# MDFahimAnjum/AliasFree-Diffusion-Models-PyTorch

Hardware: AMD Instinct MI355X
Metric: train_step_images_per_sec (higher is better)
Workload: dtype f32; 1 GPU; CIFAR-10 32x32x3 synthetic, UNet variant=3 (Config D), batch 256/GPU, T=1000, AdamW lr 3e-4, random-init weights (seed 42); global_batch=256, parallelism=dp1, hip_graph=True, launch_mode=lanes

## Files before the change

aliasfree-diffusion-models-pytorch_amd/csrc/tok.hip:

```cpp
#include "common.h"
#include <algorithm>
#include <cstdint>
#include <mutex>
#include <set>

namespace afd {

using f32x16 = __attribute__((ext_vector_type(16))) float;

template <int NB> struct TT { f32x16 b[NB]; };

__device__ __forceinline__ constexpr int tch(int j, int r) { return 32 * j + (r & 3) + 8 * (r >> 2); }

struct Pix { unsigned b, p, f; bool live; };
__device__ __forceinline__ Pix pix_of(int tile, int l31, unsigned total, unsigned P) {
  Pix q;
  q.f = (unsigned)tile * 32u + (unsigned)l31;
  q.live = q.f < total;
  const unsigned fc = q.live ? q.f : 0u;
  q.b = fc / P;
  q.p = fc - q.b * P;
  return q;
}
__device__ __forceinline__ unsigned tbase(const Pix& q, unsigned Cx, unsigned P, int half) {
  return q.b * Cx * P + q.p + 4u * (unsigned)half * P;
}

template <int NB>
__device__ __forceinline__ void t_load(TT<NB>& z, const float* __restrict__ src, unsigned base, unsigned P, bool live) {
#pragma unroll
  for (int j = 0; j < NB; ++j)
#pragma unroll
    for (int r = 0; r < 16; ++r) z.b[j][r] = live ? src[base + (unsigned)tch(j, r) * P] : 0.f;
}
template <int NB>
__device__ __forceinline__ void t_store(const TT<NB>& z, float* __restrict__ dst, unsigned base, unsigned P, bool live) {
  if (!live) return;
#pragma unroll
  for (int j = 0; j < NB; ++j)
#pragma unroll
    for (int r = 0; r < 16; ++r) dst[base + (unsigned)tch(j, r) * P] = z.b[j][r];
}

template <int KB>
__device__ __forceinline__ f32x16 t_block(const float* __restrict__ Ws, int nb, int l31, int half, const TT<KB>& z, f32x16 acc) {
  constexpr int WS = 32 * KB + 4;
  const float* __restrict__ wr = Ws + (nb * 32 + l31) * WS + 4 * half;
#pragma unroll
  for (int j = 0; j < KB; ++j)
#pragma unroll
    for (int q = 0; q < 4; ++q) {
      const float4 a = *reinterpret_cast<const float4*>(wr + 32 * j + 8 * q);
      acc = __builtin_amdgcn_mfma_f32_32x32x2f32(a.x, z.b[j][4 * q + 0], acc, 0, 0, 0);
      acc = __builtin_amdgcn_mfma_f32_32x32x2f32(a.y, z.b[j][4 * q + 1], acc, 0, 0, 0);
      acc = __builtin_amdgcn_mfma_f32_32x32x2f32(a.z, z.b[j][4 * q + 2], acc, 0, 0, 0);
      acc = __builtin_amdgcn_mfma_f32_32x32x2f32(a.w, z.b[j][4 * q + 3], acc, 0, 0, 0);
    }
  return acc;
}
__device__ __forceinline__ f32x16 zero16() {
  f32x16 a;
#pragma unroll
  for (int r = 0; r < 16; ++r) a[r] = 0.f;
  return a;
}

template <int K>
__device__ __forceinline__ void stage_w(float* __restrict__ Ws, const float* __restrict__ w, int rows, int ldw, int n0, int k0,
                                        bool transposed) {
  constexpr int WS = K + 4;
  if (!transposed) {
    for (int i = threadIdx.x; i < rows * K; i += 256) {
      const int n = i / K, k = i - n * K;
      Ws[n * WS + k] = w[(long)(n0 + n) * ldw + k0 + k];
    }
  } else {
    for (int i = threadIdx.x; i < rows * K; i += 256) {
      const int n = i / K, k = i - n * K;
      Ws[n * WS + k] = w[(long)(k0 + k) * ldw + n0 + n];
    }
  }
}

template <int KB>
__device__ __forceinline__ void t_ln_fwd(const TT<KB>& x, const float* __restrict__ gs, const float* __restrict__ bs, int half,
                                         float eps, TT<KB>& y, float& mean, float& rstd) {
  constexpr float invC = 1.0f / (32 * KB);
  float s = 0.f;
#pragma unroll
  for (int j = 0; j < KB; ++j)
#pragma unroll
    for (int r = 0; r < 16; ++r) s += x.b[j][r];
  s += __shfl_xor(s, 32, 64);
  mean = s * invC;
  float q = 0.f;
#pragma unroll
  for (int j = 0; j < KB; ++j)
#pragma unroll
    for (int r = 0; r < 16; ++r) { const float d = x.b[j][r] - mean; q = fmaf(d, d, q); }
  q += __shfl_xor(q, 32, 64);
  rstd = 1.0f / sqrtf(q * invC + eps);
#pragma unroll
  for (int j = 0; j < KB; ++j)
#pragma unroll
    for (int r = 0; r < 16; ++r) {
      const int c = tch(j, r) + 4 * half;
      y.b[j][r] = (x.b[j][r] - mean) * rstd * gs[c] + bs[c];
    }
}
template <int KB>
__device__ __forceinline__ void t_ln_bwd(TT<KB>& dy, const TT<KB>& x, const float* __restrict__ gs, int half, float mean,
                                         float rstd, const TT<KB>& add) {
  constexpr float invC = 1.0f / (32 * KB);
  float s1 = 0.f, s2 = 0.f;
#pragma unroll
  for (int j = 0; j < KB; ++j)
#pragma unroll
    for (int r = 0; r < 16; ++r) {
      const float gv = gs[tch(j, r) + 4 * half] * dy.b[j][r];
      const float xh = (x.b[j][r] - mean) * rstd;
      dy.b[j][r] = gv;
      s1 += gv;
      s2 = fmaf(gv, xh, s2);
    }
  s1 += __shfl_xor(s1, 32, 64);
  s2 += __shfl_xor(s2, 32, 64);
  const float m1 = s1 * invC, m2 = s2 * invC;
#pragma unroll
  for (int j = 0; j < KB; ++j)
#pragma unroll
    for (int r = 0; r < 16; ++r) {
      const float xh = (x.b[j][r] - mean) * rstd;
      dy.b[j][r] = rstd * (dy.b[j][r] - m1 - xh * m2) + add.b[j][r];
    }
}

template <int C>
__global__ __launch_bounds__(256) void tok_head_fwd(const float* __restrict__ x, const float* __restrict__ gamma,
                                                    const float* __restrict__ beta, const float* __restrict__ w,
                                                    const float* __restrict__ bias, float* __restrict__ h_out,
                                                    float* __restrict__ stats_out, float* __restrict__ y, int B, int N, int P,
                                                    float eps, int n_per_wg) {
  constexpr int KB = C / 32, WS = C + 4;
  extern __shared__ __attribute__((aligned(16))) float smem[];
  float* Ws = smem;
  float* bsm = Ws + n_per_wg * WS;
  float* gs = bsm + n_per_wg;
  float* bes = gs + C;
  const int nbase = blockIdx.y * n_per_wg;
  stage_w<C>(Ws, w, n_per_wg, C, nbase, 0, false);
  for (int i = threadIdx.x; i < n_per_wg; i += 256) bsm[i] = bias ? bias[nbase + i] : 0.f;
  for (int i = threadIdx.x; i < C; i += 256) { gs[i] = gamma[i]; bes[i] = beta[i]; }
  __syncthreads();

  const int lane = threadIdx.x & 63, wv = threadIdx.x >> 6, half = lane >> 5, l31 = lane & 31;
  const unsigned total = (unsigned)B * (unsigned)P;
  const int ntile = (int)((total + 31u) / 32u);
  const int tstride = gridDim.x * 4;
  const bool lead = blockIdx.y == 0;
  const int nblk = n_per_wg / 32;

  TT<KB> xc, xn;
  Pix pc, pn;
  int t = blockIdx.x * 4 + wv;
  if (t < ntile) { pc = pix_of(t, l31, total, P); t_load(xc, x, tbase(pc, C, P, half), P, pc.live); }
  for (; t < ntile; t += tstride) {
    const int tn = t + tstride;
    if (tn < ntile) { pn = pix_of(tn, l31, total, P); t_load(xn, x, tbase(pn, C, P, half), P, pn.live); }
    TT<KB> h;
    float mean, rstd;
    t_ln_fwd<KB>(xc, gs, bes, half, eps, h, mean, rstd);
    if (lead) {
      if (h_out) t_store(h, h_out, tbase(pc, C, P, half), P, pc.live);
      if (stats_out && pc.live && half == 0) { stats_out[2 * pc.f] = mean; stats_out[2 * pc.f + 1] = rstd; }
    }
    const unsigned yb = tbase(pc, N, P, half);
    for (int nb = 0; nb < nblk; ++nb) {
      const f32x16 acc = t_block<KB>(Ws, nb, l31, half, h, zero16());
      if (pc.live) {
#pragma unroll
        for (int r = 0; r < 16; ++r) {
          const int nl = nb * 32 + tch(0, r) + 4 * half;
          y[yb + (unsigned)(nbase + nb * 32 + tch(0, r)) * (unsigned)P] = acc[r] + bsm[nl];
        }
      }
    }
    xc = xn; pc = pn;
  }
}

template <int C> struct Chain {
  static constexpr int KB = C / 32, WS = C + 4, SLOT = C * WS;
  static constexpr bool RELOAD = C > 64;
  static constexpr int NSLOT = RELOAD ? 2 : 3;
};

template <int C, bool TRAIN>
__global__ __launch_bounds__(256) void tok_tail_fwd(const float* __restrict__ att, const float* __restrict__ xres,
                                                    const float* __restrict__ wo, const float* __restrict__ bo,
                                                    const float* __restrict__ gamma, const float* __restrict__ beta,
                                                    const float* __restrict__ w1, const float* __restrict__ b1,
                                                    const float* __restrict__ w2, const float* __restrict__ b2,
                                                    float* __restrict__ a_out, float* __restrict__ stats_out,
                                                    float* __restrict__ f_out, float* __restrict__ u_out, float* __restrict__ g_out,
                                                    float* __restrict__ out, int B, int P, float eps) {
  using CH = Chain<C>;
  constexpr int KB = CH::KB;
  extern __shared__ __attribute__((aligned(16))) float smem[];
  float* s0 = smem;
  float* s1 = smem + CH::SLOT;
  float* s2 = CH::RELOAD ? s0 : smem + 2 * CH::SLOT;
  float* vec = smem + CH::NSLOT * CH::SLOT;
  stage_w<C>(s0, wo, C, C, 0, 0, false);
  stage_w<C>(s1, w1, C, C, 0, 0, false);
  if (!CH::RELOAD) stage_w<C>(s2, w2, C, C, 0, 0, false);
  for (int i = threadIdx.x; i < C; i += 256) {
    vec[i] = bo[i]; vec[C + i] = gamma[i]; vec[2 * C + i] = beta[i]; vec[3 * C + i] = b1[i]; vec[4 * C + i] = b2[i];
// ... 459 lines not shown
  x_put(Xt, nbk, l31, half, dfb);
  __syncthreads();
  x_get<KB>(Xt, l31, half, z);
  const float mean = pc.live ? stats[2 * pc.f] : 0.f, rstd = pc.live ? stats[2 * pc.f + 1] : 0.f;
  float m1, m2;
  t_ln_bwd_core<KB>(z, aa, gs, half, mean, rstd, m1, m2);
  t_load(aa, dout, base, P, pc.live);
#pragma unroll
  for (int j = 0; j < KB; ++j)
#pragma unroll
    for (int r = 0; r < 16; ++r) z.b[j][r] += aa.b[j][r];
  {
    const f32x16 ab = b_load(a_in, bb, P, pc.live), dob = b_load(dout, bb, P, pc.live);
    f32x16 dab;
#pragma unroll
    for (int r = 0; r < 16; ++r) {
      const float xh = (ab[r] - mean) * rstd;
      dab[r] = rstd * (gs[cb + tch(0, r)] * dfb[r] - m1 - xh * m2) + dob[r];
    }
    b_store(dab, da_out, bb, P, pc.live);
  }
  const f32x16 db = wa_block<KB>(wa, z, zero16());
  b_store(db, datt_out, bb, P, pc.live);
}

template <int C>
__global__ __launch_bounds__(256) void tok_head_bwd_wide(const float* __restrict__ dqkv, const float* __restrict__ x,
                                                         const float* __restrict__ stats, const float* __restrict__ gamma,
                                                         const float* __restrict__ w_in, const float* __restrict__ dres,
                                                         float* __restrict__ dh_out, float* __restrict__ dx_out, int B, int P) {
  using WD = Wide<C>;
  constexpr int KB = WD::KB;
  __shared__ float X[WD::TPW][C * 32];
  __shared__ float gs[C];
  for (int i = threadIdx.x; i < C; i += 256) gs[i] = gamma[i];
  const int lane = threadIdx.x & 63, wv = threadIdx.x >> 6, half = lane >> 5, l31 = lane & 31;
  const int ts = wv / WD::NS, nbk = wv % WD::NS;
  const unsigned total = (unsigned)B * (unsigned)P;
  const int ntile = (int)((total + 31u) / 32u);
  const int tile = blockIdx.x * WD::TPW + ts;
  const bool active = tile < ntile;
  Pix pc = pix_of(active ? tile : 0, l31, total, P);
  pc.live = pc.live && active;
  const unsigned base = tbase(pc, C, P, half), bb = base + (unsigned)(nbk * 32) * (unsigned)P;
  const unsigned qb = tbase(pc, 3 * C, P, half);
  const int cb = nbk * 32 + 4 * half;
  float* Xt = X[ts];
  TT<KB> z;
  WA<KB> wa;
  f32x16 dhb = zero16();
#pragma unroll
  for (int sct = 0; sct < 3; ++sct) {
    t_load(z, dqkv, qb + (unsigned)(sct * C) * (unsigned)P, P, pc.live);
    wa_load_t(wa, w_in, nbk * 32, C, sct * C, l31, half);
    dhb = wa_block<KB>(wa, z, dhb);
  }
  if (dh_out) b_store(dhb, dh_out, bb, P, pc.live);
  x_put(Xt, nbk, l31, half, dhb);
  TT<KB> xx;
  t_load(xx, x, base, P, pc.live);
  __syncthreads();
  x_get<KB>(Xt, l31, half, z);
  const float mean = pc.live ? stats[2 * pc.f] : 0.f, rstd = pc.live ? stats[2 * pc.f + 1] : 0.f;
  float m1, m2;
  t_ln_bwd_core<KB>(z, xx, gs, half, mean, rstd, m1, m2);
  const f32x16 xb = b_load(x, bb, P, pc.live), rb = b_load(dres, bb, P, pc.live);
  f32x16 dxb;
#pragma unroll
  for (int r = 0; r < 16; ++r) {
    const float xh = (xb[r] - mean) * rstd;
    dxb[r] = rstd * (gs[cb + tch(0, r)] * dhb[r] - m1 - xh * m2) + rb[r];
  }
  b_store(dxb, dx_out, bb, P, pc.live);
}

static bool tok_ok(int C) { return C == 32 || C == 64 || C == 128; }
static size_t chain_lds(int C, int nvec) {
  const int nslot = C > 64 ? 2 : 3;
  return sizeof(float) * ((size_t)nslot * C * (C + 4) + (size_t)nvec * C);
}
template <class K> static int set_lds(K kern, size_t lds) { return lds_opt_in(kern, lds); }
static int g_tok_max_wg = 0;
static int g_tok_path = 0;
static bool use_wide(int C, long ntile) {
  if (C != 64 && C != 128) return false;
  if (g_tok_max_wg > 0 || g_tok_path == 1) return false;
  if (g_tok_path == 2) return true;
  return C == 128 || ntile < 1024;
}
static unsigned chain_grid(int C, long ntile) {
  const long wg = (ntile + 3) / 4;
  const long cap = g_tok_max_wg > 0 ? g_tok_max_wg : (C > 64 ? 8192 : 1024);
  return (unsigned)std::min<long>(wg, cap);
}

}

using namespace afd;

extern "C" {

int afd_tok_supported(int C) { return tok_ok(C) ? 1 : 0; }
int afd_debug_tok_grid(int max_workgroups) { g_tok_max_wg = max_workgroups; return AFD_OK; }
int afd_debug_tok_path(int mode) { g_tok_path = mode; return AFD_OK; }

int afd_tok_head_fwd(const float* x, const float* gamma, const float* beta, const float* w, const float* bias, float* h_out,
                     float* stats_out, float* qkv, int B, int C, int P, float eps, afd_stream_t st) {
  AFD_REQUIRE(x && gamma && beta && w && qkv && B > 0 && P > 0, "afd_tok_head_fwd: NULL pointer or empty shape");
  AFD_REQUIRE(tok_ok(C), "afd_tok_head_fwd: C=%d not covered (32, 64, 128)", C);
  AFD_REQUIRE((long)B * P * 3 * C < (1L << 31), "afd_tok_head_fwd: tensor too large for 32-bit offsets");
  const int N = 3 * C;
  const long ntile = ((long)B * P + 31) / 32, wg_tiles = (ntile + 3) / 4;
  if (use_wide(C, ntile) && aligned16(w) && (ntile <= 256 || g_tok_path == 2)) {
    const long waves = ntile * (N / 32);
    const dim3 wgrid((unsigned)((waves + 3) / 4));
    hipStream_t s = as_stream(st);
    if (C == 64) hipLaunchKernelGGL((tok_head_fwd_wide<64, 1>), wgrid, dim3(256), 0, s, x, gamma, beta, w, bias, h_out, stats_out, qkv, B, P, eps);
    else         hipLaunchKernelGGL((tok_head_fwd_wide<128, 1>), wgrid, dim3(256), 0, s, x, gamma, beta, w, bias, h_out, stats_out, qkv, B, P, eps);
    return check_launch("afd_tok_head_fwd");
  }
  int npw = 32;
  for (int cand : {N, 192, 128, 96, 64, 32}) {
    if (cand > N || N % cand != 0) continue;
    if (sizeof(float) * ((size_t)cand * (C + 5) + 2 * C) > 64 * 1024) continue;
    npw = cand;
    if (wg_tiles * (N / cand) >= 256) break;
  }
  const size_t lds = sizeof(float) * ((size_t)npw * (C + 5) + 2 * C);
  const dim3 grid((unsigned)std::min<long>(wg_tiles, g_tok_max_wg > 0 ? g_tok_max_wg : 1024), (unsigned)(N / npw));
  hipStream_t s = as_stream(st);
  switch (C) {
    case 32:  hipLaunchKernelGGL(tok_head_fwd<32>, grid, dim3(256), lds, s, x, gamma, beta, w, bias, h_out, stats_out, qkv, B, N, P, eps, npw); break;
    case 64:  hipLaunchKernelGGL(tok_head_fwd<64>, grid, dim3(256), lds, s, x, gamma, beta, w, bias, h_out, stats_out, qkv, B, N, P, eps, npw); break;
    default:  hipLaunchKernelGGL(tok_head_fwd<128>, grid, dim3(256), lds, s, x, gamma, beta, w, bias, h_out, stats_out, qkv, B, N, P, eps, npw); break;
  }
  return check_launch("afd_tok_head_fwd");
}

int afd_tok_tail_fwd(const float* att, const float* x, const float* wo, const float* bo, const float* gamma, const float* beta,
                     const float* w1, const float* b1, const float* w2, const float* b2, float* a_out, float* stats_out,
                     float* f_out, float* u_out, float* g_out, float* out, int B, int C, int P, float eps, afd_stream_t st) {
  AFD_REQUIRE(att && x && wo && bo && gamma && beta && w1 && b1 && w2 && b2 && out && B > 0 && P > 0,
              "afd_tok_tail_fwd: NULL pointer or empty shape");
  AFD_REQUIRE(tok_ok(C), "afd_tok_tail_fwd: C=%d not covered (32, 64, 128)", C);
  AFD_REQUIRE((long)B * P * C < (1L << 31), "afd_tok_tail_fwd: tensor too large for 32-bit offsets");
  const bool train = a_out != nullptr;
  AFD_REQUIRE(!train || (stats_out && f_out && u_out && g_out), "afd_tok_tail_fwd: a_out given but a saved-tensor pointer is NULL");
  const long ntile = ((long)B * P + 31) / 32;
  hipStream_t s = as_stream(st);
  if (use_wide(C, ntile) && aligned16(wo) && aligned16(w1) && aligned16(w2)) {
    const dim3 wgrid((unsigned)((ntile + Wide<64>::TPW - 1) / Wide<64>::TPW)), wgrid128((unsigned)ntile);
#define AFD_TAILW(C_, T_, G_) hipLaunchKernelGGL((tok_tail_fwd_wide<C_, T_>), G_, dim3(256), 0, s, att, x, wo, bo, gamma, beta, w1, b1, w2, b2, \
                                                  a_out, stats_out, f_out, u_out, g_out, out, B, P, eps)
    if (C == 64) { if (train) AFD_TAILW(64, true, wgrid); else AFD_TAILW(64, false, wgrid); }
    else         { if (train) AFD_TAILW(128, true, wgrid128); else AFD_TAILW(128, false, wgrid128); }
#undef AFD_TAILW
    return check_launch("afd_tok_tail_fwd");
  }
  const size_t lds = chain_lds(C, 5);
  const dim3 grid(chain_grid(C, ntile));
#define AFD_TAIL(C_, T_) do { if (int rc = set_lds(tok_tail_fwd<C_, T_>, lds)) return rc; \
    hipLaunchKernelGGL((tok_tail_fwd<C_, T_>), grid, dim3(256), lds, s, att, x, wo, bo, gamma, beta, w1, b1, w2, b2, a_out, stats_out, \
                       f_out, u_out, g_out, out, B, P, eps); } while (0)
  switch (C) {
    case 32:  if (train) AFD_TAIL(32, true); else AFD_TAIL(32, false); break;
    case 64:  if (train) AFD_TAIL(64, true); else AFD_TAIL(64, false); break;
    default:  if (train) AFD_TAIL(128, true); else AFD_TAIL(128, false); break;
  }
#undef AFD_TAIL
  return check_launch("afd_tok_tail_fwd");
}

int afd_tok_tail_bwd(const float* d_out, const float* u, const float* a, const float* stats, const float* gamma, const float* w2,
                     const float* w1, const float* wo, float* du_out, float* df_out, float* da_out, float* datt_out, int B, int C,
                     int P, afd_stream_t st) {
  AFD_REQUIRE(d_out && u && a && stats && gamma && w2 && w1 && wo && du_out && df_out && da_out && datt_out && B > 0 && P > 0,
              "afd_tok_tail_bwd: NULL pointer or empty shape");
  AFD_REQUIRE(tok_ok(C), "afd_tok_tail_bwd: C=%d not covered (32, 64, 128)", C);
  AFD_REQUIRE((long)B * P * C < (1L << 31), "afd_tok_tail_bwd: tensor too large for 32-bit offsets");
  const long ntile = ((long)B * P + 31) / 32;
  hipStream_t s = as_stream(st);
  if (use_wide(C, ntile)) {
    if (C == 64) hipLaunchKernelGGL(tok_tail_bwd_wide<64>, dim3((unsigned)((ntile + 1) / 2)), dim3(256), 0, s, d_out, u, a, stats, gamma, w2, w1, wo, du_out, df_out, da_out, datt_out, B, P);
    else         hipLaunchKernelGGL(tok_tail_bwd_wide<128>, dim3((unsigned)ntile), dim3(256), 0, s, d_out, u, a, stats, gamma, w2, w1, wo, du_out, df_out, da_out, datt_out, B, P);
    return check_launch("afd_tok_tail_bwd");
  }
  const size_t lds = chain_lds(C, 1);
  const dim3 grid(chain_grid(C, ntile));
#define AFD_TB(C_) do { if (int rc = set_lds(tok_tail_bwd<C_>, lds)) return rc; \
    hipLaunchKernelGGL(tok_tail_bwd<C_>, grid, dim3(256), lds, s, d_out, u, a, stats, gamma, w2, w1, wo, du_out, df_out, da_out, datt_out, B, P); } while (0)
  switch (C) { case 32: AFD_TB(32); break; case 64: AFD_TB(64); break; default: AFD_TB(128); break; }
#undef AFD_TB
  return check_launch("afd_tok_tail_bwd");
}

int afd_tok_head_bwd(const float* dqkv, const float* x, const float* stats, const float* gamma, const float* w_in,
                     const float* d_res, float* dh_out, float* dx_out, int B, int C, int P, afd_stream_t st) {
  AFD_REQUIRE(dqkv && x && stats && gamma && w_in && d_res && dx_out && B > 0 && P > 0, "afd_tok_head_bwd: NULL pointer or empty shape");
  AFD_REQUIRE(tok_ok(C), "afd_tok_head_bwd: C=%d not covered (32, 64, 128)", C);
  AFD_REQUIRE((long)B * P * 3 * C < (1L << 31), "afd_tok_head_bwd: tensor too large for 32-bit offsets");
  const long ntile = ((long)B * P + 31) / 32;
  hipStream_t s = as_stream(st);
  if (use_wide(C, ntile)) {
    if (C == 64) hipLaunchKernelGGL(tok_head_bwd_wide<64>, dim3((unsigned)((ntile + 1) / 2)), dim3(256), 0, s, dqkv, x, stats, gamma, w_in, d_res, dh_out, dx_out, B, P);
    else         hipLaunchKernelGGL(tok_head_bwd_wide<128>, dim3((unsigned)ntile), dim3(256), 0, s, dqkv, x, stats, gamma, w_in, d_res, dh_out, dx_out, B, P);
    return check_launch("afd_tok_head_bwd");
  }
  const size_t lds = chain_lds(C, 1);
  const dim3 grid(chain_grid(C, ntile));
#define AFD_HB(C_) do { if (int rc = set_lds(tok_head_bwd<C_>, lds)) return rc; \
    hipLaunchKernelGGL(tok_head_bwd<C_>, grid, dim3(256), lds, s, dqkv, x, stats, gamma, w_in, d_res, dh_out, dx_out, B, P); } while (0)
  switch (C) { case 32: AFD_HB(32); break; case 64: AFD_HB(64); break; default: AFD_HB(128); break; }
#undef AFD_HB
  return check_launch("afd_tok_head_bwd");
}

}
```

Baseline: 38070 images/s.

## Route token-MLP kernels through split-fp16 MFMA path for C=64/128

Adds a new family of token head/tail forward and backward kernels that split f32 activations and weights into hi/lo fp16 pairs with per-row scaling. The matmuls run as three f16 32x32x16 MFMAs per block, approximating f32 precision, in place of the f32 32x32x2 MFMA. Weights are staged once per workgroup as fp16 images in LDS across persistent passes. The path is enabled by default for C=64/128 when the tile count is large enough. It trades the f32 MFMA throughput limit for extra split and scale arithmetic and a small loss of precision compared to exact f32.

```diff
diff --git a/aliasfree-diffusion-models-pytorch_amd/csrc/tok.hip b/aliasfree-diffusion-models-pytorch_amd/csrc/tok.hip
--- a/aliasfree-diffusion-models-pytorch_amd/csrc/tok.hip
+++ b/aliasfree-diffusion-models-pytorch_amd/csrc/tok.hip
@@ -1,46 +1,11 @@
-#include "common.h"
+#include "tok_common.h"
+#include "tok_h2.h"
 #include <algorithm>
 #include <cstdint>
 #include <mutex>
 #include <set>
 
 namespace afd {
-
-using f32x16 = __attribute__((ext_vector_type(16))) float;
-
-template <int NB> struct TT { f32x16 b[NB]; };
-
-__device__ __forceinline__ constexpr int tch(int j, int r) { return 32 * j + (r & 3) + 8 * (r >> 2); }
-
-struct Pix { unsigned b, p, f; bool live; };
-__device__ __forceinline__ Pix pix_of(int tile, int l31, unsigned total, unsigned P) {
-  Pix q;
-  q.f = (unsigned)tile * 32u + (unsigned)l31;
-  q.live = q.f < total;
-  const unsigned fc = q.live ? q.f : 0u;
-  q.b = fc / P;
-  q.p = fc - q.b * P;
-  return q;
-}
-__device__ __forceinline__ unsigned tbase(const Pix& q, unsigned Cx, unsigned P, int half) {
-  return q.b * Cx * P + q.p + 4u * (unsigned)half * P;
-}
-
-template <int NB>
-__device__ __forceinline__ void t_load(TT<NB>& z, const float* __restrict__ src, unsigned base, unsigned P, bool live) {
-#pragma unroll
-  for (int j = 0; j < NB; ++j)
-#pragma unroll
-    for (int r = 0; r < 16; ++r) z.b[j][r] = live ? src[base + (unsigned)tch(j, r) * P] : 0.f;
-}
-template <int NB>
-__device__ __forceinline__ void t_store(const TT<NB>& z, float* __restrict__ dst, unsigned base, unsigned P, bool live) {
-  if (!live) return;
-#pragma unroll
-  for (int j = 0; j < NB; ++j)
-#pragma unroll
-    for (int r = 0; r < 16; ++r) dst[base + (unsigned)tch(j, r) * P] = z.b[j][r];
-}
 
 template <int KB>
 __device__ __forceinline__ f32x16 t_block(const float* __restrict__ Ws, int nb, int l31, int half, const TT<KB>& z, f32x16 acc) {
@@ -57,12 +22,6 @@
       acc = __builtin_amdgcn_mfma_f32_32x32x2f32(a.w, z.b[j][4 * q + 3], acc, 0, 0, 0);
     }
   return acc;
-}
-__device__ __forceinline__ f32x16 zero16() {
-  f32x16 a;
-#pragma unroll
-  for (int r = 0; r < 16; ++r) a[r] = 0.f;
-  return a;
 }
 
 template <int K>
@@ -80,59 +39,6 @@
       Ws[n * WS + k] = w[(long)(k0 + k) * ldw + n0 + n];
     }
   }
-}
-
-template <int KB>
-__device__ __forceinline__ void t_ln_fwd(const TT<KB>& x, const float* __restrict__ gs, const float* __restrict__ bs, int half,
-                                         float eps, TT<KB>& y, float& mean, float& rstd) {
-  constexpr float invC = 1.0f / (32 * KB);
-  float s = 0.f;
-#pragma unroll
-  for (int j = 0; j < KB; ++j)
-#pragma unroll
-    for (int r = 0; r < 16; ++r) s += x.b[j][r];
-  s += __shfl_xor(s, 32, 64);
-  mean = s * invC;
-  float q = 0.f;
-#pragma unroll
-  for (int j = 0; j < KB; ++j)
-#pragma unroll
-    for (int r = 0; r < 16; ++r) { const float d = x.b[j][r] - mean; q = fmaf(d, d, q); }
-  q += __shfl_xor(q, 32, 64);
-  rstd = 1.0f / sqrtf(q * invC + eps);
-#pragma unroll
-  for (int j = 0; j < KB; ++j)
-#pragma unroll
-    for (int r = 0; r < 16; ++r) {
-      const int c = tch(j, r) + 4 * half;
-      y.b[j][r] = (x.b[j][r] - mean) * rstd * gs[c] + bs[c];
-    }
-}
-template <int KB>
-__device__ __forceinline__ void t_ln_bwd(TT<KB>& dy, const TT<KB>& x, const float* __restrict__ gs, int half, float mean,
-                                         float rstd, const TT<KB>& add) {
-  constexpr float invC = 1.0f / (32 * KB);
-  float s1 = 0.f, s2 = 0.f;
-#pragma unroll
-  for (int j = 0; j < KB; ++j)
-#pragma unroll
-    for (int r = 0; r < 16; ++r) {
-      const float gv = gs[tch(j, r) + 4 * half] * dy.b[j][r];
-      const float xh = (x.b[j][r] - mean) * rstd;
-      dy.b[j][r] = gv;
-      s1 += gv;
-      s2 = fmaf(gv, xh, s2);
-    }
-  s1 += __shfl_xor(s1, 32, 64);
-  s2 += __shfl_xor(s2, 32, 64);
-  const float m1 = s1 * invC, m2 = s2 * invC;
-#pragma unroll
-  for (int j = 0; j < KB; ++j)
-#pragma unroll
-    for (int r = 0; r < 16; ++r) {
-      const float xh = (x.b[j][r] - mean) * rstd;
-      dy.b[j][r] = rstd * (dy.b[j][r] - m1 - xh * m2) + add.b[j][r];
-    }
 }
 
 template <int C>
@@ -758,6 +664,13 @@
 template <class K> static int set_lds(K kern, size_t lds) { return lds_opt_in(kern, lds); }
 static int g_tok_max_wg = 0;
 static int g_tok_path = 0;
+static bool use_h2(int C, long ntile, int kern) {
+  if (C != 64 && C != 128) return false;
+  if (g_tok_path >= 4) return true;
+  if (g_tok_path != 0) return false;
+  if (C == 64) return ntile >= 1024 || (kern == 2 && ntile >= 512);
+  return kern != 1 && ntile >= 512;
+}
 static bool use_wide(int C, long ntile) {
   if (C != 64 && C != 128) return false;
   if (g_tok_max_wg > 0 || g_tok_path == 1) return false;
@@ -778,7 +691,12 @@
 
 int afd_tok_supported(int C) { return tok_ok(C) ? 1 : 0; }
 int afd_debug_tok_grid(int max_workgroups) { g_tok_max_wg = max_workgroups; return AFD_OK; }
-int afd_debug_tok_path(int mode) { g_tok_path = mode; return AFD_OK; }
+int afd_debug_tok_path(int mode) {
+  AFD_REQUIRE(mode >= 0 && mode <= 6, "afd_debug_tok_path: mode %d not in 0..6", mode);
+  g_tok_path = mode;
+  tok_h2_debug_tpw(mode == 5 ? 2 : (mode == 6 ? 4 : 0));
+  return AFD_OK;
+}
 
 int afd_tok_head_fwd(const float* x, const float* gamma, const float* beta, const float* w, const float* bias, float* h_out,
                      float* stats_out, float* qkv, int B, int C, int P, float eps, afd_stream_t st) {
@@ -787,6 +705,7 @@
   AFD_REQUIRE((long)B * P * 3 * C < (1L << 31), "afd_tok_head_fwd: tensor too large for 32-bit offsets");
   const int N = 3 * C;
   const long ntile = ((long)B * P + 31) / 32, wg_tiles = (ntile + 3) / 4;
+  if (use_h2(C, ntile, 0)) return tok_h2_head_fwd(x, gamma, beta, w, bias, h_out, stats_out, qkv, B, C, P, eps, g_tok_max_wg, as_stream(st));
   if (use_wide(C, ntile) && aligned16(w) && (ntile <= 256 || g_tok_path == 2)) {
     const long waves = ntile * (N / 32);
     const dim3 wgrid((unsigned)((waves + 3) / 4));
@@ -824,6 +743,8 @@
   AFD_REQUIRE(!train || (stats_out && f_out && u_out && g_out), "afd_tok_tail_fwd: a_out given but a saved-tensor pointer is NULL");
   const long ntile = ((long)B * P + 31) / 32;
   hipStream_t s = as_stream(st);
+  if (use_h2(C, ntile, 1))
+    return tok_h2_tail_fwd(att, x, wo, bo, gamma, beta, w1, b1, w2, b2, a_out, stats_out, f_out, u_out, g_out, out, B, C, P, eps, g_tok_max_wg, s);
   if (use_wide(C, ntile) && aligned16(wo) && aligned16(w1) && aligned16(w2)) {
     const dim3 wgrid((unsigned)((ntile + Wide<64>::TPW - 1) / Wide<64>::TPW)), wgrid128((unsigned)ntile);
 #define AFD_TAILW(C_, T_, G_) hipLaunchKernelGGL((tok_tail_fwd_wide<C_, T_>), G_, dim3(256), 0, s, att, x, wo, bo, gamma, beta, w1, b1, w2, b2, \
@@ -856,6 +777,7 @@
   AFD_REQUIRE((long)B * P * C < (1L << 31), "afd_tok_tail_bwd: tensor too large for 32-bit offsets");
   const long ntile = ((long)B * P + 31) / 32;
   hipStream_t s = as_stream(st);
+  if (use_h2(C, ntile, 2)) return tok_h2_tail_bwd(d_out, u, a, stats, gamma, w2, w1, wo, du_out, df_out, da_out, datt_out, B, C, P, g_tok_max_wg, s);
   if (use_wide(C, ntile)) {
     if (C == 64) hipLaunchKernelGGL(tok_tail_bwd_wide<64>, dim3((unsigned)((ntile + 1) / 2)), dim3(256), 0, s, d_out, u, a, stats, gamma, w2, w1, wo, du_out, df_out, da_out, datt_out, B, P);
     else         hipLaunchKernelGGL(tok_tail_bwd_wide<128>, dim3((unsigned)ntile), dim3(256), 0, s, d_out, u, a, stats, gamma, w2, w1, wo, du_out, df_out, da_out, datt_out, B, P);
@@ -877,6 +799,7 @@
   AFD_REQUIRE((long)B * P * 3 * C < (1L << 31), "afd_tok_head_bwd: tensor too large for 32-bit offsets");
   const long ntile = ((long)B * P + 31) / 32;
   hipStream_t s = as_stream(st);
+  if (use_h2(C, ntile, 3)) return tok_h2_head_bwd(dqkv, x, stats, gamma, w_in, d_res, dh_out, dx_out, B, C, P, g_tok_max_wg, s);
   if (use_wide(C, ntile)) {
     if (C == 64) hipLaunchKernelGGL(tok_head_bwd_wide<64>, dim3((unsigned)((ntile + 1) / 2)), dim3(256), 0, s, dqkv, x, stats, gamma, w_in, d_res, dh_out, dx_out, B, P);
     else         hipLaunchKernelGGL(tok_head_bwd_wide<128>, dim3((unsigned)ntile), dim3(256), 0, s, dqkv, x, stats, gamma, w_in, d_res, dh_out, dx_out, B, P);
diff --git a/aliasfree-diffusion-models-pytorch_amd/csrc/tok_common.h b/aliasfree-diffusion-models-pytorch_amd/csrc/tok_common.h
--- /dev/null
+++ b/aliasfree-diffusion-models-pytorch_amd/csrc/tok_common.h
@@ -0,0 +1,102 @@
+#pragma once
+#include "common.h"
+
+namespace afd {
+
+using f32x16 = __attribute__((ext_vector_type(16))) float;
+
+template <int NB> struct TT { f32x16 b[NB]; };
+
+__device__ __forceinline__ constexpr int tch(int j, int r) { return 32 * j + (r & 3) + 8 * (r >> 2); }
+
+struct Pix { unsigned b, p, f; bool live; };
+__device__ __forceinline__ Pix pix_of(int tile, int l31, unsigned total, unsigned P) {
+  Pix q;
+  q.f = (unsigned)tile * 32u + (unsigned)l31;
+  q.live = q.f < total;
+  const unsigned fc = q.live ? q.f : 0u;
+  q.b = fc / P;
+  q.p = fc - q.b * P;
+  return q;
+}
+__device__ __forceinline__ unsigned tbase(const Pix& q, unsigned Cx, unsigned P, int half) {
+  return q.b * Cx * P + q.p + 4u * (unsigned)half * P;
+}
+
+template <int NB>
+__device__ __forceinline__ void t_load(TT<NB>& z, const float* __restrict__ src, unsigned base, unsigned P, bool live) {
+#pragma unroll
+  for (int j = 0; j < NB; ++j)
+#pragma unroll
+    for (int r = 0; r < 16; ++r) z.b[j][r] = live ? src[base + (unsigned)tch(j, r) * P] : 0.f;
+}
+template <int NB>
+__device__ __forceinline__ void t_store(const TT<NB>& z, float* __restrict__ dst, unsigned base, unsigned P, bool live) {
+  if (!live) return;
+#pragma unroll
+  for (int j = 0; j < NB; ++j)
+#pragma unroll
+    for (int r = 0; r < 16; ++r) dst[base + (unsigned)tch(j, r) * P] = z.b[j][r];
+}
+
+__device__ __forceinline__ f32x16 zero16() {
+  f32x16 a;
+#pragma unroll
+  for (int r = 0; r < 16; ++r) a[r] = 0.f;
+  return a;
+}
+
+template <int KB>
+__device__ __forceinline__ void t_ln_fwd(const TT<KB>& x, const float* __restrict__ gs, const float* __restrict__ bs, int half,
+                                         float eps, TT<KB>& y, float& mean, float& rstd) {
+  constexpr float invC = 1.0f / (32 * KB);
+  float s = 0.f;
+#pragma unroll
+  for (int j = 0; j < KB; ++j)
+#pragma unroll
+    for (int r = 0; r < 16; ++r) s += x.b[j][r];
+  s += __shfl_xor(s, 32, 64);
+  mean = s * invC;
+  float q = 0.f;
+#pragma unroll
+  for (int j = 0; j < KB; ++j)
+#pragma unroll
+    for (int r = 0; r < 16; ++r) { const float d = x.b[j][r] - mean; q = fmaf(d, d, q); }
+  q += __shfl_xor(q, 32, 64);
+  rstd = 1.0f / sqrtf(q * invC + eps);
+#pragma unroll
+  for (int j = 0; j < KB; ++j)
+#pragma unroll
+    for (int r = 0; r < 16; ++r) {
+      const int c = tch(j, r) + 4 * half;
+      y.b[j][r] = (x.b[j][r] - mean) * rstd * gs[c] + bs[c];
+    }
+}
+template <int KB>
+__device__ __forceinline__ void t_ln_bwd(TT<KB>& dy, const TT<KB>& x, const float* __restrict__ gs, int half, float mean,
+                                         float rstd, const TT<KB>& add) {
+  constexpr float invC = 1.0f / (32 * KB);
+  float s1 = 0.f, s2 = 0.f;
+#pragma unroll
+  for (int j = 0; j < KB; ++j)
+#pragma unroll
+    for (int r = 0; r < 16; ++r) {
+      const float gv = gs[tch(j, r) + 4 * half] * dy.b[j][r];
+      const float xh = (x.b[j][r] - mean) * rstd;
+      dy.b[j][r] = gv;
+      s1 += gv;
+      s2 = fmaf(gv, xh, s2);
+    }
+  s1 += __shfl_xor(s1, 32, 64);
+  s2 += __shfl_xor(s2, 32, 64);
+  const float m1 = s1 * invC, m2 = s2 * invC;
+#pragma unroll
+  for (int j = 0; j < KB; ++j)
+#pragma unroll
+    for (int r = 0; r < 16; ++r) {
+      const float xh = (x.b[j][r] - mean) * rstd;
+      dy.b[j][r] = rstd * (dy.b[j][r] - m1 - xh * m2) + add.b[j][r];
+    }
+}
+
+}
diff --git a/aliasfree-diffusion-models-pytorch_amd/csrc/tok_h2.h b/aliasfree-diffusion-models-pytorch_amd/csrc/tok_h2.h
--- /dev/null
+++ b/aliasfree-diffusion-models-pytorch_amd/csrc/tok_h2.h
@@ -0,0 +1,18 @@
+#pragma once
+#include "common.h"
+
+namespace afd {
+
+int tok_h2_head_fwd(const float* x, const float* gamma, const float* beta, const float* w, const float* bias, float* h_out,
+                    float* stats_out, float* qkv, int B, int C, int P, float eps, int max_wg, hipStream_t s);
+int tok_h2_tail_fwd(const float* att, const float* x, const float* wo, const float* bo, const float* gamma, const float* beta,
+                    const float* w1, const float* b1, const float* w2, const float* b2, float* a_out, float* stats_out,
+                    float* f_out, float* u_out, float* g_out, float* out, int B, int C, int P, float eps, int max_wg, hipStream_t s);
+int tok_h2_tail_bwd(const float* d_out, const float* u, const float* a, const float* stats, const float* gamma, const float* w2,
+                    const float* w1, const float* wo, float* du_out, float* df_out, float* da_out, float* datt_out, int B, int C,
+                    int P, int max_wg, hipStream_t s);
+int tok_h2_head_bwd(const float* dqkv, const float* x, const float* stats, const float* gamma, const float* w_in,
+                    const float* d_res, float* dh_out, float* dx_out, int B, int C, int P, int max_wg, hipStream_t s);
+void tok_h2_debug_tpw(int tpw);
+
+}
diff --git a/aliasfree-diffusion-models-pytorch_amd/csrc/tok_h2.hip b/aliasfree-diffusion-models-pytorch_amd/csrc/tok_h2.hip
--- /dev/null
+++ b/aliasfree-diffusion-models-pytorch_amd/csrc/tok_h2.hip
@@ -0,0 +1,526 @@
+#include "tok_common.h"
+#include "h2_common.h"
+#include "tok_h2.h"
+#include <algorithm>
+
+namespace afd {
+
+template <int NB>
+__device__ __forceinline__ void h_load(TT<NB>& z, const float* __restrict__ src, unsigned base, int P) {
+#pragma unroll
+  for (int j = 0; j < NB; ++j)
+#pragma unroll
+    for (int r = 0; r < 16; ++r) z.b[j][r] = (src + (size_t)tch(j, r) * P)[base];
+}
+template <int NB>
+__device__ __forceinline__ void h_store(const TT<NB>& z, float* __restrict__ dst, unsigned base, int P, bool live) {
+  if (!live) return;
+#pragma unroll
+  for (int j = 0; j < NB; ++j)
+#pragma unroll
+    for (int r = 0; r < 16; ++r) (dst + (size_t)tch(j, r) * P)[base] = z.b[j][r];
+}
+
+template <int KB> struct HP { h8 a[2 * KB], b[2 * KB]; };
+
+template <int KB>
+__device__ __forceinline__ float hp_split(const TT<KB>& z, HP<KB>& p) {
+  float m = 0.f;
+#pragma unroll
+  for (int j = 0; j < KB; ++j)
+#pragma unroll
+    for (int r = 0; r < 16; ++r) m = fmaxf(m, fabsf(z.b[j][r]));
+  m = fmaxf(m, __shfl_xor(m, 32, 64));
+  const float s = h2_scale_for(m);
+#pragma unroll
+  for (int k = 0; k < 2 * KB; ++k) {
+    float x[8];
+#pragma unroll
+    for (int e = 0; e < 8; ++e) x[e] = z.b[k >> 1][8 * (k & 1) + e];
+    h2_split8(x, s, p.a[k], p.b[k]);
+  }
+  return h2_inv_pow2(s);
+}
+
+template <int KB>
+__device__ __forceinline__ f32x16 hp_block(const h8* __restrict__ img, int nb, int l31, int half, const HP<KB>& z) {
+  constexpr int C = 32 * KB, NG = C / 8;
+  const h8* __restrict__ w0 = img + half * C + nb * 32 + l31;
+  const h8* __restrict__ w1 = w0 + NG * C;
+  f32x16 acc = zero16();
+#pragma unroll
+  for (int k = 0; k < 2 * KB; ++k) {
+    const h8 a1 = w0[2 * k * C], a2 = w1[2 * k * C];
+    acc = __builtin_amdgcn_mfma_f32_32x32x16_f16(a2, z.a[k], acc, 0, 0, 0);
+    acc = __builtin_amdgcn_mfma_f32_32x32x16_f16(a1, z.b[k], acc, 0, 0, 0);
+    acc = __builtin_amdgcn_mfma_f32_32x32x16_f16(a1, z.a[k], acc, 0, 0, 0);
+  }
+  return acc;
+}
+
+template <int C> struct H2Lds {
+  static constexpr int NG = C / 8, REC = 2 * NG * C;
+  static constexpr bool RELOAD = C > 64;
+  static constexpr int NSLOT = RELOAD ? 2 : 3;
+  h8* img[3];
+  float* winv[3];
+  unsigned* rmax[3];
+  float* vec;
+  __device__ __forceinline__ void init(unsigned char* base) {
+    h8* i0 = reinterpret_cast<h8*>(base);
+    float* w0 = reinterpret_cast<float*>(i0 + NSLOT * REC);
+    unsigned* r0 = reinterpret_cast<unsigned*>(w0 + NSLOT * C);
+#pragma unroll
+    for (int m = 0; m < 3; ++m) {
+      const int s = m % NSLOT;
+      img[m] = i0 + s * REC; winv[m] = w0 + s * C; rmax[m] = r0 + s * C;
+    }
+    vec = reinterpret_cast<float*>(r0 + NSLOT * C);
+  }
+  static size_t bytes(int nvec) { return (size_t)NSLOT * REC * 16 + (size_t)NSLOT * C * 8 + (size_t)nvec * C * 4; }
+};
+
+struct WSrc { const float* w; int ldw, n0, k0; };
+
+template <int C, int NT> struct Stg {
+  static constexpr int NG = C / 8, NR = C * NG / NT;
+  float x[NR][8];
+  static __device__ __forceinline__ void rec(int r, bool transposed, int& n, int& G) {
+    const int i = (int)threadIdx.x + r * NT;
+    if (transposed) { n = i % C; G = i / C; }
+    else {
+      const int lo = i & 63, hi = i >> 6;
+      n = (hi % (C / 8)) * 8 + (lo & 7);
+      G = (hi / (C / 8)) * 8 + (lo >> 3);
+    }
+  }
+  __device__ __forceinline__ void load(const WSrc& q, bool transposed) {
+#pragma unroll
+    for (int r = 0; r < NR; ++r) {
+      int n, G;
+      rec(r, transposed, n, G);
+      const int kb = 16 * (G >> 1) + 4 * (G & 1);
+#pragma unroll
+      for (int e = 0; e < 8; ++e) {
+        const int k = kb + 8 * (e >> 2) + (e & 3);
+        x[r][e] = transposed ? q.w[(long)(q.k0 + k) * q.ldw + q.n0 + n] : q.w[(long)(q.n0 + n) * q.ldw + q.k0 + k];
+      }
+    }
+  }
+  __device__ __forceinline__ void maxima(unsigned* __restrict__ rmax, bool transposed) const {
+#pragma unroll
+    for (int r = 0; r < NR; ++r) {
+      int n, G;
+      rec(r, transposed, n, G);
+      float m = 0.f;
+#pragma unroll
+      for (int e = 0; e < 8; ++e) m = fmaxf(m, fabsf(x[r][e]));
+      atomicMax(&rmax[n], __float_as_uint(m));
+    }
+  }
+  __device__ __forceinline__ void store(h8* __restrict__ img, float* __restrict__ winv, const unsigned* __restrict__ rmax,
+                                        bool transposed) const {
+#pragma unroll
+    for (int r = 0; r < NR; ++r) {
+      int n, G;
+      rec(r, transposed, n, G);
+      const float sc = h2_scale_for(__uint_as_float(rmax[n]));
+      h8 p0, p1;
+      h2_split8(x[r], sc, p0, p1);
+      img[G * C + n] = p0;
+      img[(NG + G) * C + n] = p1;
+      if (G == 0) winv[n] = h2_inv_pow2(sc);
+    }
+  }
+};
+
+template <int C, int NT, int M0, int CNT>
+__device__ __forceinline__ void h2_stage(const H2Lds<C>& L, const WSrc* src, bool transposed) {
+  Stg<C, NT> st[CNT];
+#pragma unroll
+  for (int i = 0; i < CNT; ++i) st[i].load(src[i], transposed);
+#pragma unroll
+  for (int i = 0; i < CNT; ++i)
+    for (int c = threadIdx.x; c < C; c += NT) L.rmax[M0 + i][c] = 0u;
+  __syncthreads();
+#pragma unroll
+  for (int i = 0; i < CNT; ++i) st[i].maxima(L.rmax[M0 + i], transposed);
+  __syncthreads();
+#pragma unroll
+  for (int i = 0; i < CNT; ++i) st[i].store(L.img[M0 + i], L.winv[M0 + i], L.rmax[M0 + i], transposed);
+  __builtin_amdgcn_sched_barrier(0);
+}
+template <int C, int NT>
+__device__ __forceinline__ void h2_stage_first(const H2Lds<C>& L, const WSrc* src, bool transposed) {
+  if (H2Lds<C>::RELOAD) h2_stage<C, NT, 0, 2>(L, src, transposed);
+  else h2_stage<C, NT, 0, 3>(L, src, transposed);
+}
+template <int C, int NT, int M>
+__device__ __forceinline__ void h2_stage_one(const H2Lds<C>& L, const WSrc* src, bool transposed) {
+  h2_stage<C, NT, M, 1>(L, src + M, transposed);
+}
+
+struct Walk { int lane, wv, half, l31, ntile, tstride, t0, npass; unsigned total; };
+template <int TPW> __device__ __forceinline__ Walk walk_of(int B, int P) {
+  Walk k;
+  k.lane = threadIdx.x & 63; k.wv = threadIdx.x >> 6; k.half = k.lane >> 5; k.l31 = k.lane & 31;
+  k.total = (unsigned)B * (unsigned)P;
+  k.ntile = (int)((k.total + 31u) / 32u);
+  k.tstride = gridDim.x * TPW;
+  k.t0 = blockIdx.x * TPW;
+  k.npass = k.t0 < k.ntile ? (k.ntile - k.t0 + k.tstride - 1) / k.tstride : 0;
+  return k;
+}
+
+extern __shared__ __attribute__((aligned(16))) unsigned char h2_smem[];
+
+template <int C, int TPW>
+__global__ __launch_bounds__(64 * TPW) void tok_h2_head_fwd_k(const float* __restrict__ x, const float* __restrict__ gamma,
+                                                               const float* __restrict__ beta, const float* __restrict__ w,
+                                                               const float* __restrict__ bias, float* __restrict__ h_out,
+                                                               float* __restrict__ stats_out, float* __restrict__ y, int B, int P,
+                                                               float eps) {
+  using LD = H2Lds<C>;
+  constexpr int KB = C / 32, NT = 64 * TPW;
+  LD L;
+  L.init(h2_smem);
+  float* vec = L.vec;
+  const Walk k = walk_of<TPW>(B, P);
+  const int half = k.half, l31 = k.l31;
+  const WSrc src[3] = {{w, C, 0, 0}, {w, C, C, 0}, {w, C, 2 * C, 0}};
+  h2_stage_first<C, NT>(L, src, false);
+  for (int i = threadIdx.x; i < C; i += NT) { vec[i] = gamma[i]; vec[C + i] = beta[i]; }
+  for (int i = threadIdx.x; i < 3 * C; i += NT) vec[2 * C + i] = bias ? bias[i] : 0.f;
+  __syncthreads();
+  for (int pass = 0; pass < k.npass; ++pass) {
+    const int t = k.t0 + k.wv + pass * k.tstride;
+    const bool active = t < k.ntile;
+    if (LD::RELOAD && pass > 0) { __syncthreads(); h2_stage_one<C, NT, 0>(L, src, false); __syncthreads(); }
+    Pix pc = pix_of(active ? t : 0, l31, k.total, P);
+    pc.live = pc.live && active;
+    const unsigned yb = tbase(pc, 3 * C, P, half);
+    HP<KB> hp;
+    float is = 0.f;
+    if (active) {
+      const unsigned base = tbase(pc, C, P, half);
+      TT<KB> xc, h;
+      h_load(xc, x, base, P);
+      float mean, rstd;
+      t_ln_fwd<KB>(xc, vec, vec + C, half, eps, h, mean, rstd);
+      if (h_out) h_store(h, h_out, base, P, pc.live);
+      if (stats_out && pc.live && half == 0) { stats_out[2 * pc.f] = mean; stats_out[2 * pc.f + 1] = rstd; }
+      is = hp_split<KB>(h, hp);
+    }
+#pragma unroll
+    for (int sl = 0; sl < 3; ++sl) {
+      if (LD::RELOAD && sl == 1) { __syncthreads(); h2_stage_one<C, NT, 2>(L, src, false); }
+      if (LD::RELOAD && sl == 2) __syncthreads();
+      if (active) {
+#pragma unroll
+        for (int nb = 0; nb < KB; ++nb) {
+          const f32x16 acc = hp_block<KB>(L.img[sl], nb, l31, half, hp);
+          if (pc.live) {
+#pragma unroll
+            for (int r = 0; r < 16; ++r) {
+              const int c = nb * 32 + tch(0, r) + 4 * half;
+              (y + (size_t)(sl * C + nb * 32 + tch(0, r)) * P)[yb] = acc[r] * is * L.winv[sl][c] + vec[2 * C + sl * C + c];
+            }
+          }
+        }
+      }
+    }
+  }
+}
+
+template <int C, int TPW, bool TRAIN>
+__global__ __launch_bounds__(64 * TPW) void tok_h2_tail_fwd_k(const float* __restrict__ att, const float* __restrict__ xres,
+                                                               const float* __restrict__ wo, const float* __restrict__ bo,
+                                                               const float* __restrict__ gamma, const float* __restrict__ beta,
+                                                               const float* __restrict__ w1, const float* __restrict__ b1,
+                                                               const float* __restrict__ w2, const float* __restrict__ b2,
+                                                               float* __restrict__ a_out, float* __restrict__ stats_out,
+                                                               float* __restrict__ f_out, float* __restrict__ u_out,
+                                                               float* __restrict__ g_out, float* __restrict__ out, int B, int P,
+                                                               float eps) {
+  using LD = H2Lds<C>;
+  constexpr int KB = C / 32, NT = 64 * TPW;
+  LD L;
+  L.init(h2_smem);
+  float* vec = L.vec;
+  const Walk k = walk_of<TPW>(B, P);
+  const int half = k.half, l31 = k.l31;
+  const WSrc src[3] = {{wo, C, 0, 0}, {w1, C, 0, 0}, {w2, C, 0, 0}};
+  h2_stage_first<C, NT>(L, src, false);
+  for (int i = threadIdx.x; i < C; i += NT) {
+    vec[i] = bo[i]; vec[C + i] = gamma[i]; vec[2 * C + i] = beta[i]; vec[3 * C + i] = b1[i]; vec[4 * C + i] = b2[i];
+  }
+  __syncthreads();
+  for (int pass = 0; pass < k.npass; ++pass) {
+    const int t = k.t0 + k.wv + pass * k.tstride;
+    const bool active = t < k.ntile;
+    if (LD::RELOAD && pass > 0) { __syncthreads(); h2_stage_one<C, NT, 0>(L, src, false); __syncthreads(); }
+    Pix pc = pix_of(active ? t : 0, l31, k.total, P);
+    pc.live = pc.live && active;
+    const unsigned base = tbase(pc, C, P, half);
+    TT<KB> a;
+    HP<KB> hp;
+    float is = 0.f;
+    if (active) {
+      TT<KB> z, xr;
+      h_load(z, att, base, P);
+      h_load(xr, xres, base, P);
+      is = hp_split<KB>(z, hp);
+#pragma unroll
+      for (int nb = 0; nb < KB; ++nb) {
+        const f32x16 acc = hp_block<KB>(L.img[0], nb, l31, half, hp);
+#pragma unroll
+        for (int r = 0; r < 16; ++r) {
+          const int c = nb * 32 + tch(0, r) + 4 * half;
+          a.b[nb][r] = acc[r] * is * L.winv[0][c] + vec[c] + xr.b[nb][r];
+        }
+      }
+      float mean, rstd;
+      t_ln_fwd<KB>(a, vec + C, vec + 2 * C, half, eps, z, mean, rstd);
+      if (TRAIN) {
+        h_store(a, a_out, base, P, pc.live);
+        h_store(z, f_out, base, P, pc.live);
+        if (pc.live && half == 0) { stats_out[2 * pc.f] = mean; stats_out[2 * pc.f + 1] = rstd; }
+      }
+      is = hp_split<KB>(z, hp);
+    }
+    if (LD::RELOAD) { __syncthreads(); h2_stage_one<C, NT, 2>(L, src, false); }
+    if (active) {
+      TT<KB> g;
+#pragma unroll
+      for (int nb = 0; nb < KB; ++nb) {
+        const f32x16 acc = hp_block<KB>(L.img[1], nb, l31, half, hp);
+        TT<1> ub;
+#pragma unroll
+        for (int r = 0; r < 16; ++r) {
+          const int c = nb * 32 + tch(0, r) + 4 * half;
+          ub.b[0][r] = acc[r] * is * L.winv[1][c] + vec[3 * C + c];
+          g.b[nb][r] = gelu_erf(ub.b[0][r]);
+        }
+        if (TRAIN) h_store(ub, u_out + (size_t)(32 * nb) * P, base, P, pc.live);
+      }
+      if (TRAIN) h_store(g, g_out, base, P, pc.live);
+      is = hp_split<KB>(g, hp);
+    }
+    if (LD::RELOAD) __syncthreads();
+    if (active) {
+#pragma unroll
+      for (int nb = 0; nb < KB; ++nb) {
+        TT<1> ar;
+        if (TRAIN && KB > 2) h_load(ar, a_out + (size_t)(32 * nb) * P, base, P);
+        else ar.b[0] = a.b[nb];
+        const f32x16 acc = hp_block<KB>(L.img[2], nb, l31, half, hp);
+        if (pc.live) {
+#pragma unroll
+          for (int r = 0; r < 16; ++r) {
+            const int c = nb * 32 + tch(0, r) + 4 * half;
+            (out + (size_t)tch(nb, r) * P)[base] = acc[r] * is * L.winv[2][c] + vec[4 * C + c] + ar.b[0][r];
+          }
+        }
+      }
+    }
+  }
+}
+
+template <int C, int TPW>
+__global__ __launch_bounds__(64 * TPW) void tok_h2_tail_bwd_k(const float* __restrict__ dout, const float* __restrict__ u_in,
+                                                               const float* __restrict__ a_in, const float* __restrict__ stats,
+                                                               const float* __restrict__ gamma, const float* __restrict__ w2,
+                                                               const float* __restrict__ w1, const float* __restrict__ wo,
+                                                               float* __restrict__ du_out, float* __restrict__ df_out,
+                                                               float* __restrict__ da_out, float* __restrict__ datt_out, int B,
+                                                               int P) {
+  using LD = H2Lds<C>;
+  constexpr int KB = C / 32, NT = 64 * TPW;
+  LD L;
+  L.init(h2_smem);
+  float* gs = L.vec;
+  const Walk k = walk_of<TPW>(B, P);
+  const int half = k.half, l31 = k.l31;
+  const WSrc src[3] = {{w2, C, 0, 0}, {w1, C, 0, 0}, {wo, C, 0, 0}};
+  h2_stage_first<C, NT>(L, src, true);
+  for (int i = threadIdx.x; i < C; i += NT) gs[i] = gamma[i];
+  __syncthreads();
+  for (int pass = 0; pass < k.npass; ++pass) {
+    const int t = k.t0 + k.wv + pass * k.tstride;
+    const bool active = t < k.ntile;
+    if (LD::RELOAD && pass > 0) { __syncthreads(); h2_stage_one<C, NT, 0>(L, src, true); __syncthreads(); }
+    Pix pc = pix_of(active ? t : 0, l31, k.total, P);
+    pc.live = pc.live && active;
+    const unsigned base = tbase(pc, C, P, half);
+    HP<KB> hp;
+    float is = 0.f;
+    if (active) {
+      TT<KB> z, uu;
+      h_load(z, dout, base, P);
+      h_load(uu, u_in, base, P);
+      is = hp_split<KB>(z, hp);
+#pragma unroll
+      for (int nb = 0; nb < KB; ++nb) {
+        const f32x16 acc = hp_block<KB>(L.img[0], nb, l31, half, hp);
+#pragma unroll
+        for (int r = 0; r < 16; ++r)
+          z.b[nb][r] = acc[r] * is * L.winv[0][nb * 32 + tch(0, r) + 4 * half] * gelu_erf_grad(uu.b[nb][r]);
+      }
+      h_store(z, du_out, base, P, pc.live);
+      is = hp_split<KB>(z, hp);
+    }
+    if (LD::RELOAD) { __syncthreads(); h2_stage_one<C, NT, 2>(L, src, true); }
+    if (active) {
+      TT<KB> df, aa, dd;
+#pragma unroll
+      for (int nb = 0; nb < KB; ++nb) {
+        const f32x16 acc = hp_block<KB>(L.img[1], nb, l31, half, hp);
+#pragma unroll
+        for (int r = 0; r < 16; ++r) df.b[nb][r] = acc[r] * is * L.winv[1][nb * 32 + tch(0, r) + 4 * half];
+      }
+      h_store(df, df_out, base, P, pc.live);
+      h_load(dd, dout, base, P);
+      h_load(aa, a_in, base, P);
+      const float mean = pc.live ? stats[2 * pc.f] : 0.f, rstd = pc.live ? stats[2 * pc.f + 1] : 0.f;
+      t_ln_bwd<KB>(df, aa, gs, half, mean, rstd, dd);
+      h_store(df, da_out, base, P, pc.live);
+      is = hp_split<KB>(df, hp);
+    }
+    if (LD::RELOAD) __syncthreads();
+    if (active) {
+#pragma unroll
+      for (int nb = 0; nb < KB; ++nb) {
+        const f32x16 acc = hp_block<KB>(L.img[2], nb, l31, half, hp);
+        if (pc.live) {
+#pragma unroll
+          for (int r = 0; r < 16; ++r)
+            (datt_out + (size_t)tch(nb, r) * P)[base] = acc[r] * is * L.winv[2][nb * 32 + tch(0, r) + 4 * half];
+        }
+      }
+    }
+  }
+}
+
+template <int C, int TPW>
+__global__ __launch_bounds__(64 * TPW) void tok_h2_head_bwd_k(const float* __restrict__ dqkv, const float* __restrict__ x,
+                                                               const float* __restrict__ stats, const float* __restrict__ gamma,
+                                                               const float* __restrict__ w_in, const float* __restrict__ dres,
+                                                               float* __restrict__ dh_out, float* __restrict__ dx_out, int B,
+                                                               int P) {
+  using LD = H2Lds<C>;
+  constexpr int KB = C / 32, NT = 64 * TPW;
+  LD L;
+  L.init(h2_smem);
+  float* gs = L.vec;
+  const Walk k = walk_of<TPW>(B, P);
+  const int half = k.half, l31 = k.l31;
+  const WSrc src[3] = {{w_in, C, 0, 0}, {w_in, C, 0, C}, {w_in, C, 0, 2 * C}};
+  h2_stage_first<C, NT>(L, src, true);
+  for (int i = threadIdx.x; i < C; i += NT) gs[i] = gamma[i];
+  __syncthreads();
+  for (int pass = 0; pass < k.npass; ++pass) {
+    const int t = k.t0 + k.wv + pass * k.tstride;
+    const bool active = t < k.ntile;
+    if (LD::RELOAD && pass > 0) { __syncthreads(); h2_stage_one<C, NT, 0>(L, src, true); __syncthreads(); }
+    Pix pc = pix_of(active ? t : 0, l31, k.total, P);
+    pc.live = pc.live && active;
+    const unsigned base = tbase(pc, C, P, half);
+    const unsigned qb = tbase(pc, 3 * C, P, half);
+    TT<KB> dh;
+#pragma unroll
+    for (int sl = 0; sl < 3; ++sl) {
+      if (LD::RELOAD && sl == 1) { __syncthreads(); h2_stage_one<C, NT, 2>(L, src, true); }
+      if (LD::RELOAD && sl == 2) __syncthreads();
+      if (active) {
+        TT<KB> z;
+        HP<KB> hp;
+        h_load(z, dqkv + (size_t)(sl * C) * P, qb, P);
+        const float is = hp_split<KB>(z, hp);
+#pragma unroll
+        for (int nb = 0; nb < KB; ++nb) {
+          const f32x16 acc = hp_block<KB>(L.img[sl], nb, l31, half, hp);
+#pragma unroll
+          for (int r = 0; r < 16; ++r) {
+            const float v = acc[r] * is * L.winv[sl][nb * 32 + tch(0, r) + 4 * half];
+            dh.b[nb][r] = sl == 0 ? v : dh.b[nb][r] + v;
+          }
+        }
+      }
+    }
+    if (active) {
+      if (dh_out) h_store(dh, dh_out, base, P, pc.live);
+      TT<KB> xx, rr;
+      h_load(xx, x, base, P);
+      h_load(rr, dres, base, P);
+      const float mean = pc.live ? stats[2 * pc.f] : 0.f, rstd = pc.live ? stats[2 * pc.f + 1] : 0.f;
+      t_ln_bwd<KB>(dh, xx, gs, half, mean, rstd, rr);
+      h_store(dh, dx_out, base, P, pc.live);
+    }
+  }
+}
+
+static int g_h2_tpw = 0;
+void tok_h2_debug_tpw(int tpw) { g_h2_tpw = tpw; }
+static int h2_tpw(long ntile) { (void)ntile; return g_h2_tpw ? g_h2_tpw : 4; }
+static unsigned h2_grid(int C, long ntile, int tpw, int max_wg) {
+  const long wg = (ntile + tpw - 1) / tpw;
+  const long cap = max_wg > 0 ? max_wg : (C > 64 ? 256 : 768);
+  return (unsigned)std::min<long>(wg, cap);
+}
+
+#define AFD_H2_LAUNCH(KERN, NVEC, ...)                                                                              \
+  do {                                                                                                              \
+    const size_t lds = H2Lds<KC>::bytes(NVEC);                                                                      \
+    if (int rc = lds_opt_in(KERN, lds)) return rc;                                                                  \
+    hipLaunchKernelGGL(KERN, dim3(h2_grid(KC, ntile, KT, max_wg)), dim3(64 * KT), lds, s, __VA_ARGS__);             \
+  } while (0)
+#define AFD_H2_SWITCH(BODY)                                                                                         \
+  do {                                                                                                              \
+    if (C == 64) { constexpr int KC = 64; if (tpw == 4) { constexpr int KT = 4; BODY; } else { constexpr int KT = 2; BODY; } } \
+    else         { constexpr int KC = 128; constexpr int KT = 4; BODY; }                                             \
+  } while (0)
+
+int tok_h2_head_fwd(const float* x, const float* gamma, const float* beta, const float* w, const float* bias, float* h_out,
+                    float* stats_out, float* qkv, int B, int C, int P, float eps, int max_wg, hipStream_t s) {
+  const long ntile = ((long)B * P + 31) / 32;
+  const int tpw = h2_tpw(ntile);
+  AFD_H2_SWITCH(AFD_H2_LAUNCH((tok_h2_head_fwd_k<KC, KT>), 5, x, gamma, beta, w, bias, h_out, stats_out, qkv, B, P, eps));
+  return check_launch("afd_tok_head_fwd");
+}
+
+int tok_h2_tail_fwd(const float* att, const float* x, const float* wo, const float* bo, const float* gamma, const float* beta,
+                    const float* w1, const float* b1, const float* w2, const float* b2, float* a_out, float* stats_out,
+                    float* f_out, float* u_out, float* g_out, float* out, int B, int C, int P, float eps, int max_wg, hipStream_t s) {
+  const long ntile = ((long)B * P + 31) / 32;
+  const int tpw = h2_tpw(ntile);
+  if (a_out)
+    AFD_H2_SWITCH(AFD_H2_LAUNCH((tok_h2_tail_fwd_k<KC, KT, true>), 5, att, x, wo, bo, gamma, beta, w1, b1, w2, b2, a_out, stats_out,
+                                f_out, u_out, g_out, out, B, P, eps));
+  else
+    AFD_H2_SWITCH(AFD_H2_LAUNCH((tok_h2_tail_fwd_k<KC, KT, false>), 5, att, x, wo, bo, gamma, beta, w1, b1, w2, b2, a_out, stats_out,
+                                f_out, u_out, g_out, out, B, P, eps));
+  return check_launch("afd_tok_tail_fwd");
+}
+
+int tok_h2_tail_bwd(const float* d_out, const float* u, const float* a, const float* stats, const float* gamma, const float* w2,
+                    const float* w1, const float* wo, float* du_out, float* df_out, float* da_out, float* datt_out, int B, int C,
+                    int P, int max_wg, hipStream_t s) {
+  const long ntile = ((long)B * P + 31) / 32;
+  const int tpw = h2_tpw(ntile);
+  AFD_H2_SWITCH(AFD_H2_LAUNCH((tok_h2_tail_bwd_k<KC, KT>), 1, d_out, u, a, stats, gamma, w2, w1, wo, du_out, df_out, da_out, datt_out,
+                              B, P));
+  return check_launch("afd_tok_tail_bwd");
+}
+
+int tok_h2_head_bwd(const float* dqkv, const float* x, const float* stats, const float* gamma, const float* w_in,
+                    const float* d_res, float* dh_out, float* dx_out, int B, int C, int P, int max_wg, hipStream_t s) {
+  const long ntile = ((long)B * P + 31) / 32;
+  const int tpw = h2_tpw(ntile);
+  AFD_H2_SWITCH(AFD_H2_LAUNCH((tok_h2_head_bwd_k<KC, KT>), 1, dqkv, x, stats, gamma, w_in, d_res, dh_out, dx_out, B, P));
+  return check_launch("afd_tok_head_bwd");
+}
+
+#undef AFD_H2_SWITCH
+#undef AFD_H2_LAUNCH
+
+}
```

After: 38690 images/s, median of 6. +1.6%, better.
